# uzh-rpg/rpg_svo

Measured on AMD Instinct MI355X. Metric: frames/sec sparse-align+pose-refine (VGA, 4 pyr lvls); ATE vs CPU ref, higher is better.
Workload: dtype value = default build: K1 f32 pixels/residuals/chi2/per-pixel products, f64 Jacobian rows/partials/reductions/projection/solve/pose; K4 f64 (reference-width build: roofline_f64_build.value)

## Files before the change

rpg_svo_amd/csrc/pyr_addr.h:

```cpp
#pragma once
#include <stdint.h>

#ifndef SVO_HOST_MATH_TEST
#include <hip/hip_runtime.h>
#endif

namespace svo_pyr {

constexpr int TILE_W = 16, TILE_H = 8;

__host__ __device__ __forceinline__ uint32_t mul24(uint32_t a, uint32_t b) {
#ifdef __HIP_DEVICE_COMPILE__
  return __umul24(a, b);
#else
  return a * b;
#endif
}

__host__ __device__ __forceinline__ uint32_t row_off(int y, int pitch) {
  return mul24((uint32_t)(y >> 3), ((uint32_t)pitch << 3) - 128u) + ((uint32_t)y << 4);
}
__host__ __device__ __forceinline__ uint32_t col_off(int x) {
  return mul24((uint32_t)(x >> 4), 112u) + (uint32_t)x;
}
__host__ __device__ __forceinline__ uint32_t px_off(int x, int y, int pitch) { return row_off(y, pitch) + col_off(x); }

__host__ __device__ __forceinline__ int64_t level_bytes(int pitch, int h) {
  return (int64_t)pitch * ((h + 7) & ~7);
}


__device__ __forceinline__ int run_start(int c, int need) {
  int xa = c & ~3;
  if ((xa & 15) == 8 && (c & 15) + need <= 16) xa -= 4;
  return xa;
}

typedef uint32_t u32x2_t __attribute__((ext_vector_type(2)));
typedef uint32_t u32x3_t __attribute__((ext_vector_type(3)));
__device__ __forceinline__ uint32_t ld32(const uint8_t* __restrict__ lvl, uint32_t off) {
  return *reinterpret_cast<const uint32_t*>(lvl + off);
}
__device__ __forceinline__ u32x2_t ld64(const uint8_t* __restrict__ lvl, uint32_t off) {
  typedef u32x2_t __attribute__((aligned(4))) u32x2_a4;
  return *reinterpret_cast<const u32x2_a4*>(lvl + off);
}
__device__ __forceinline__ u32x3_t ld96(const uint8_t* __restrict__ lvl, uint32_t off) {
  typedef u32x3_t __attribute__((aligned(4))) u32x3_a4;
  return *reinterpret_cast<const u32x3_a4*>(lvl + off);
}

__device__ __forceinline__ void load_run12(const uint8_t* __restrict__ lvl, uint32_t ro, int xa, uint32_t d[3]) {
  const uint32_t a = ro + col_off(xa);
  const int o = xa & 15;
  if (o <= 4) {
    const u32x3_t v = ld96(lvl, a);
    d[0] = v.x; d[1] = v.y; d[2] = v.z;
  } else if (o == 8) {
    const u32x2_t v = ld64(lvl, a);
    d[0] = v.x; d[1] = v.y;
    d[2] = ld32(lvl, a + 120u);
  } else {
    d[0] = ld32(lvl, a);
    const u32x2_t v = ld64(lvl, a + 116u);
    d[1] = v.x; d[2] = v.y;
  }
}

template <int NR>
__device__ __forceinline__ void load_window12(const uint8_t* __restrict__ lvl, int pitch, int xa, int v0,
                                              uint32_t d[][3]) {
  uint32_t a[NR];
  const uint32_t c = col_off(xa);
#pragma unroll
  for (int r = 0; r < NR; ++r) a[r] = row_off(v0 + r, pitch) + c;
  const int o = xa & 15;
  if (o <= 4) {
#pragma unroll
    for (int r = 0; r < NR; ++r) {
      const u32x3_t v = ld96(lvl, a[r]);
      d[r][0] = v.x; d[r][1] = v.y; d[r][2] = v.z;
    }
  } else if (o == 8) {
#pragma unroll
    for (int r = 0; r < NR; ++r) {
      const u32x2_t v = ld64(lvl, a[r]);
      d[r][0] = v.x; d[r][1] = v.y;
      d[r][2] = ld32(lvl, a[r] + 120u);
    }
  } else {
#pragma unroll
    for (int r = 0; r < NR; ++r) {
      d[r][0] = ld32(lvl, a[r]);
      const u32x2_t v = ld64(lvl, a[r] + 116u);
      d[r][1] = v.x; d[r][2] = v.y;
    }
  }
}

}
```

rpg_svo_amd/csrc/sia_common.h:

```cpp
#pragma once
#include "capi_common.h"
#include "device_math.h"
#include "track_math.h"
#include "wave_reduce.h"

namespace svo_sia {

using namespace svo_capi;
using namespace svo_dev;

struct SiaArgs {
  svo_hip_pyr_layout L;
  const uint8_t* store;
  const int32_t* ref_slot;
  const int32_t* cur_slot;
  const int32_t* n;
  int n_stride;
  const double* px;
  const double* xyz;
  const uint8_t* valid;
  svo_hip_sia_params P;
  const double* T_in;
  double* T_out;
  double* H_out;
  int32_t* n_tracked;
  int32_t* iters;
  double* chi2;
  int32_t* status;
  int B = 0;
  void* xw = nullptr;
};

struct XChunk {
  unsigned lo, tag0, hi, tag1;
};
static_assert(sizeof(XChunk) == 16, "one 16-byte access");
constexpr int SIA_X_SLOTS = 16;
constexpr int SIA_XH_SLOTS = 24;
constexpr int SIA_X_MAX_PARTS = 4;
constexpr int SIA_X_CHUNKS = 2 * SIA_X_MAX_PARTS * (SIA_X_SLOTS + SIA_XH_SLOTS);
constexpr int SIA_X_BLOCK = SIA_X_CHUNKS + 1;

#ifndef SVO_HOST_MATH_TEST
__device__ __forceinline__ void sia_xstore(XChunk* p, double v, unsigned epoch) {
  typedef unsigned int u4 __attribute__((ext_vector_type(4)));
  const unsigned long long b = (unsigned long long)__double_as_longlong(v);
  u4 w;
  w.x = (unsigned)b; w.y = epoch; w.z = (unsigned)(b >> 32); w.w = epoch;
  asm volatile("global_store_dwordx4 %0, %1, off sc1\n\ts_nop 3" ::"v"(p), "v"(w) : "memory");
}
__device__ __forceinline__ XChunk sia_xload(const XChunk* p) {
  typedef unsigned int u4 __attribute__((ext_vector_type(4)));
  u4 w;
  asm volatile("global_load_dwordx4 %0, %1, off sc1\n\ts_waitcnt vmcnt(0)" : "=v"(w) : "v"(p) : "memory");
  XChunk c;
  c.lo = w.x; c.tag0 = w.y; c.hi = w.z; c.tag1 = w.w;
  return c;
}
__device__ __forceinline__ void sia_xstore_epoch(XChunk* p, unsigned epoch) {
  typedef unsigned int u4 __attribute__((ext_vector_type(4)));
  u4 w;
  w.x = epoch; w.y = 0u; w.z = 0u; w.w = 0u;
  asm volatile("global_store_dwordx4 %0, %1, off sc1\n\ts_nop 3" ::"v"(p), "v"(w) : "memory");
}
__device__ __forceinline__ double sia_xpoll(const XChunk* p, unsigned epoch, int& failed) {
  XChunk c = sia_xload(p);
  unsigned spins = 0;
  while (c.tag0 != epoch || c.tag1 != epoch) {
    if (++spins > (1u << 16)) {
      failed = 1;
      return __longlong_as_double(0x7ff8000000000000ll);
    }
    __builtin_amdgcn_s_sleep(1);
    c = sia_xload(p);
  }
  return __longlong_as_double((long long)(((unsigned long long)c.hi << 32) | c.lo));
}
#endif

using svo_pyr::load_window12;
using svo_pyr::run_start;


__device__ __forceinline__ void cut_row7(const uint32_t d[3], uint32_t bo, float out[7]) {
  const bool up = bo >= 4u;
  const uint32_t a = up ? d[1] : d[0], b = up ? d[2] : d[1], c = up ? 0u : d[2];
  const uint32_t sel = bo & 3u;
  const uint32_t lo = __builtin_amdgcn_alignbyte(b, a, sel);
  const uint32_t hi = __builtin_amdgcn_alignbyte(c, b, sel);
  out[0] = (float)(lo & 0xffu);
  out[1] = (float)((lo >> 8) & 0xffu);
  out[2] = (float)((lo >> 16) & 0xffu);
  out[3] = (float)(lo >> 24);
  out[4] = (float)(hi & 0xffu);
  out[5] = (float)((hi >> 8) & 0xffu);
  out[6] = (float)((hi >> 16) & 0xffu);
}

__device__ __forceinline__ void cut_row5_plain(const uint32_t d[3], uint32_t bo, float out[5]) {
  const bool up = bo >= 4u;
  const uint32_t a = up ? d[1] : d[0], b = up ? d[2] : d[1];
  const uint32_t sel = bo & 3u;
  const uint32_t lo = __builtin_amdgcn_alignbyte(b, a, sel);
  const uint32_t hi = b >> (8 * sel);
  out[0] = (float)(lo & 0xffu);
  out[1] = (float)((lo >> 8) & 0xffu);
  out[2] = (float)((lo >> 16) & 0xffu);
  out[3] = (float)(lo >> 24);
  out[4] = (float)(hi & 0xffu);
}

__device__ __forceinline__ double sia_rcp(double z) {
  double r = __builtin_amdgcn_rcp(z);
  r = fma(fma(-z, r, 1.0), r, r);
  r = fma(fma(-z, r, 1.0), r, r);
  return r;
}

__device__ __forceinline__ uint32_t sel_e64(uint64_t mask, uint32_t if_set, uint32_t if_clear) {
#ifdef SIA_VCC_SELECT
  return ((mask >> (threadIdx.x & 63)) & 1) ? if_set : if_clear;
#else
  uint32_t r;
  asm("v_cndmask_b32_e64 %0, %1, %2, %3" : "=v"(r) : "v"(if_clear), "v"(if_set), "s"(mask));
  return r;
#endif
}
__device__ __forceinline__ void cut_row5(uint32_t a, uint32_t b, uint32_t c, int bo, uint64_t up, float out[5]) {
  const uint32_t d0 = sel_e64(up, b, a), d1 = sel_e64(up, c, b);
  const uint32_t sel = (uint32_t)(bo & 3);
  const uint32_t lo = __builtin_amdgcn_alignbyte(d1, d0, sel);
  const uint32_t hi = d1 >> (8 * sel);
  out[0] = (float)(lo & 0xffu);
  out[1] = (float)((lo >> 8) & 0xffu);
  out[2] = (float)((lo >> 16) & 0xffu);
  out[3] = (float)(lo >> 24);
  out[4] = (float)(hi & 0xffu);
}

__device__ __forceinline__ double sia_uni(double v) {
  const unsigned long long u = (unsigned long long)__double_as_longlong(v);
  const unsigned lo = (unsigned)__builtin_amdgcn_readfirstlane((int)(unsigned)u);
  const unsigned hi = (unsigned)__builtin_amdgcn_readfirstlane((int)(unsigned)(u >> 32));
  return __longlong_as_double((long long)(((unsigned long long)hi << 32) | lo));
}


__device__ __forceinline__ int sym6_rt(int i, int j) {
  const int a = i < j ? i : j, b = i < j ? j : i;
  return a * 6 - (a * (a - 1)) / 2 + (b - a);
}

int launch_sia_wave(const SiaArgs& args, int B, hipStream_t s);
bool sia_wave_applies(const SiaArgs& args, int B);

}
```

rpg_svo_amd/csrc/sparse_align.hip:

```cpp
#include <cstdlib>
#include <map>
#include <mutex>
#include <utility>

#include "sia_common.h"

using namespace svo_capi;
using namespace svo_dev;
using namespace svo_sia;

namespace {

#define MINW(BLOCK) ((BLOCK) >= 256 ? 4 : 3)

#ifdef SIA_PROFILE
#define SIA_T() ((long long)__builtin_readcyclecounter())
#define SIA_ACC(k, t0, t1) prof[k] += (t1) - (t0)
#else
#define SIA_T() 0ll
#define SIA_ACC(k, t0, t1)
#endif

constexpr int MAX_WAVES = SVO_HIP_MAX_PATCHES / 64;

// ... 6 lines not shown
using sia_pix = float;
using sia_acc = double;
#endif

struct SplitModel {
  double q[2][4], t[2][3];
};

struct SiaLds {
  SplitModel sm;
  double Rt[12];
  int sw_done, sw_stop, sw_nmeas, sw_cur, sw_old;
  double sw_chi2;
  double H[21];
  double Hinv[36];
  double A[36];
  sia_acc part[2][MAX_WAVES][8];
  int chg[2][MAX_WAVES];
  int xfail;
  sia_acc Hpart[MAX_WAVES][24];
  long long lo[SVO_HIP_MAX_LEVELS];
  int lw[SVO_HIP_MAX_LEVELS];
  int lh[SVO_HIP_MAX_LEVELS];
  int lp[SVO_HIP_MAX_LEVELS];
};
__shared__ SiaLds g_s;


template <int PARTS>
__device__ __forceinline__ void sia_rebuild_hinv(int lane, int nw, [[maybe_unused]] XChunk* xh, [[maybe_unused]] int part,
                                                 [[maybe_unused]] unsigned gen, [[maybe_unused]] int& xfail) {
  asm volatile("" : "+v"(lane));
#ifndef SVO_HOST_MATH_TEST
  if constexpr (PARTS > 1) {
    static_assert((PARTS - 1) * 21 <= 64, "one lane per chunk of the other parts");
    const int j = lane / 21, k = lane - 21 * j;
    double v = 0.0;
    for (int w = 0; w < nw; ++w) v += (double)g_s.Hpart[w][k];
    if (j == 0) sia_xstore(xh + part * SIA_XH_SLOTS + k, v, gen);
    const int other = j < part ? j : j + 1;
    double got = 0.0;
    if (j < PARTS - 1) got = sia_xpoll(xh + other * SIA_XH_SLOTS + k, gen, xfail);
    if (xfail) g_s.xfail = 1;
    double tot = 0.0;
#pragma unroll
    for (int p = 0; p < PARTS; ++p) {
      const double theirs = __shfl(got, (p < part ? p : p - 1) * 21 + k, 64);
      const double term = p == part ? v : theirs;
      tot = p == 0 ? term : tot + term;
    }
    if (lane < 21) g_s.H[lane] = tot;
  } else
#endif
  if (lane < 21) {
    double v = 0.0;
    for (int w = 0; w < nw; ++w) v += (double)g_s.Hpart[w][lane];
    g_s.H[lane] = v;
  }
  SVO_WAVE_LDS_FENCE();
  const int gi = lane / 6, gj = lane - 6 * gi;
  if (lane < 36) {
    g_s.A[lane] = g_s.H[sym6_rt(gi, gj)];
    g_s.Hinv[lane] = (gi == gj) ? 1.0 : 0.0;
  }
  for (int k = 0; k < 6; ++k) {
    SVO_WAVE_LDS_FENCE();
    if (lane < 36) {
      const double p = g_s.A[k * 6 + k];
      const double aik = g_s.A[gi * 6 + k];
      const double akj = g_s.A[k * 6 + gj];
      const double bkj = g_s.Hinv[k * 6 + gj];
      const double aij = g_s.A[lane];
      const double bij = g_s.Hinv[lane];
      const double ip = (fabs(p) > 2.2250738585072014e-308) ? sia_rcp(p) : 0.0;
      const double na = (gi == k) ? akj * ip : aij - aik * (akj * ip);
      const double nb = (gi == k) ? bkj * ip : bij - aik * (bkj * ip);
      SVO_LANES_LDS_FENCE();
      g_s.A[lane] = na;
      g_s.Hinv[lane] = nb;
    }
  }
}


__device__ __forceinline__ float sia_bilerp(float wtl, float wtr, float wbl, float wbr, float tl, float tr, float bl, float br) {
  return __builtin_fmaf(wbr, br, __builtin_fmaf(wbl, bl, __builtin_fmaf(wtr, tr, wtl * tl)));
}
typedef float sia_f2 __attribute__((ext_vector_type(2)));
__device__ __forceinline__ sia_f2 sia_bilerp2(sia_f2 wtl, sia_f2 wtr, sia_f2 wbl, sia_f2 wbr, sia_f2 tl, sia_f2 tr, sia_f2 bl,
                                              sia_f2 br) {
  return __builtin_elementwise_fma(wbr, br, __builtin_elementwise_fma(wbl, bl, __builtin_elementwise_fma(wtr, tr, wtl * tl)));
}

#ifdef SIA_F64_PARTIALS
#define SIA_PACKED 0
#else
#define SIA_PACKED 1
#endif
template <int BLOCK, bool WC, bool DIST, int PARTS = 1>
__global__ void __launch_bounds__(BLOCK, PARTS > 1 ? 1 : ((DIST && BLOCK < 1024) ? 3 : MINW(BLOCK))) sia_kernel(const SiaArgs a) {
  constexpr int NW = BLOCK / 64;
  int b, part = 0;
  if constexpr (PARTS > 1) {
    b = (int)(blockIdx.x / (8 * PARTS)) * 8 + (int)(blockIdx.x % 8);
    part = (int)(blockIdx.x / 8) % PARTS;
    if (b >= a.B) return;
  } else {
    b = (int)xcd_contiguous_block();
  }
  [[maybe_unused]] XChunk* const xbase = PARTS > 1 ? static_cast<XChunk*>(a.xw) + (size_t)b * SIA_X_BLOCK : nullptr;
  [[maybe_unused]] unsigned xseq = 0;
#ifndef SVO_HOST_MATH_TEST
  if constexpr (PARTS > 1) xseq = (unsigned)__builtin_amdgcn_readfirstlane((int)sia_xload(xbase + SIA_X_CHUNKS).lo);
#endif
  [[maybe_unused]] int xfail = 0;
  const int tid = threadIdx.x;
  const int lane = tid & 63;
  const int wave = tid >> 6;

  __shared__ float4 s_bt[8][BLOCK];

  int n = a.n[b];
  n = n > a.n_stride ? a.n_stride : n;
  const svo_hip_sia_params P = a.P;

  if (n <= 0) {
    if (tid == 0 && part == 0) {
      for (int k = 0; k < 12; ++k) a.T_out[12 * b + k] = a.T_in[12 * b + k];
      if (a.H_out)
        for (int k = 0; k < 36; ++k) a.H_out[36 * b + k] = 0.0;
      a.n_tracked[b] = 0;
      if (a.iters)
        for (int k = 0; k < SVO_HIP_MAX_LEVELS; ++k) a.iters[SVO_HIP_MAX_LEVELS * b + k] = 0;
      if (a.chi2) a.chi2[b] = 1e10;
      if (a.status) a.status[b] = 0;
    }
    return;
  }

  const int pid = part * BLOCK + tid;
  const size_t fo = (size_t)b * a.n_stride + pid;
  const bool has = (pid < n) && (a.valid ? a.valid[fo] != 0 : true);
  double X = 0, Y = 0, Z = 1;
  if (has) {
    X = a.xyz[3 * fo];
    Y = a.xyz[3 * fo + 1];
    Z = a.xyz[3 * fo + 2];
  }
  double px_kept0 = 0, px_kept1 = 0;
  if (has) {
    px_kept0 = a.px[2 * fo];
    px_kept1 = a.px[2 * fo + 1];
  }
  const double rz = sia_rcp(Z);
  const sia_acc zi = (sia_acc)rz;
  const sia_acc xn = (sia_acc)(X * rz);
  const sia_acc yn = (sia_acc)(Y * rz);
  const uint8_t* ref_base = a.store + (int64_t)a.ref_slot[b] * a.L.slot_bytes;
  const uint8_t* cur_base = a.store + (int64_t)a.cur_slot[b] * a.L.slot_bytes;

  if (tid == 0) {
#pragma unroll
    for (int k = 0; k < SVO_HIP_MAX_LEVELS; ++k) {
      g_s.lw[k] = a.L.w[k];
      g_s.lh[k] = a.L.h[k];
      g_s.lp[k] = a.L.pitch[k];
      g_s.lo[k] = a.L.offset[k];
    }
    for (int k = 0; k < 21; ++k) g_s.H[k] = 0.0;
    g_s.xfail = 0;
    if (a.iters && part == 0)
      for (int k = 0; k < SVO_HIP_MAX_LEVELS; ++k) a.iters[SVO_HIP_MAX_LEVELS * b + k] = 0;
  }
  double R[9], tr[3];
  {
    double q[4];
    for (int k = 0; k < 9; ++k) R[k] = a.T_in[12 * b + k];
    for (int k = 0; k < 3; ++k) tr[k] = a.T_in[12 * b + 9 + k];
    quat_from_R(R, q);
    quat_to_R(q, R);
    if (tid == 0) {
      for (int k = 0; k < 4; ++k) g_s.sm.q[0][k] = q[k];
      for (int k = 0; k < 3; ++k) g_s.sm.t[0][k] = tr[k];
    }
  }
  int m_cur = 0, m_old = 0;
  double chi2_prev = 1e10;
  int stop = 0;
  int n_meas_last = 0;
  int buf = 0;

  const int sw = (NW > 1) ? (int)(blockIdx.x % NW) : 0;
  sia_pix Sxx = 0, Sxy = 0, Syy = 0;
  sia_acc gmask = 0;
  bool vis = false;

  __syncthreads();

#ifdef SIA_PROFILE
  long long prof[8] = {0, 0, 0, 0, 0, 0, 0, 0};
  const long long t_begin = SIA_T();
#endif
  for (int level = P.max_level; level >= P.min_level; --level) {
    [[maybe_unused]] const long long tl0 = SIA_T();
    const int cols = g_s.lw[level], rows = g_s.lh[level], pitch = g_s.lp[level];
    const uint8_t* ref_img = ref_base + g_s.lo[level];
    const uint8_t* cur_img = cur_base + g_s.lo[level];
    const float scale = pow2_inv_f32(level);
    const sia_acc fl = (sia_acc)(fabs(P.fx) * pow2_inv_f64(level));

    uint32_t wc[WC ? 7 : 1][3];
    int wc_u0 = 0, wc_v0 = -100000;
    if (WC) {
#pragma unroll
      for (int r = 0; r < (WC ? 7 : 1); ++r) wc[r][0] = wc[r][1] = wc[r][2] = 0u;
    }
    {
      const double pxx = px_kept0, pxy = px_kept1;
      const float u_ref = (float)(pxx * (double)scale);
      const float v_ref = (float)(pxy * (double)scale);
      const int u_i = (int)floorf(u_ref);
      const int v_i = (int)floorf(v_ref);
      const bool inb = has && !(u_i - 3 < 0 || v_i - 3 < 0 || u_i + 3 >= cols || v_i + 3 >= rows);
      Sxx = Sxy = Syy = 0;
      if (inb) {
        vis = true;
        gmask = 1;
        const float su = u_ref - (float)u_i, sv = v_ref - (float)v_i;
        const float wtl = (1.f - su) * (1.f - sv);
        const float wtr = su * (1.f - sv);
        const float wbl = (1.f - su) * sv;
        const float wbr = su * sv;
        float Bt[6][6];
        float Wp[7], Wc[7];
        uint32_t rw[7][3];
        const int rxa = run_start(u_i - 3, 7);
        const uint32_t rbo = (uint32_t)(u_i - 3 - rxa);
        load_window12<7>(ref_img, pitch, rxa, v_i - 3, rw);
        cut_row7(rw[0], rbo, Wp);
#pragma unroll
        for (int r = 0; r < 6; ++r) {
          cut_row7(rw[r + 1], rbo, Wc);
#pragma unroll
          for (int c = 0; c < 6; ++c) {
            const bool need = ((r >= 1 && r <= 4)) || ((c >= 1 && c <= 4));
            if (need) Bt[r][c] = sia_bilerp(wtl, wtr, wbl, wbr, Wp[c], Wp[c + 1], Wc[c], Wc[c + 1]);
          }
#pragma unroll
          for (int c = 0; c < 7; ++c) Wp[c] = Wc[c];
        }
#pragma unroll
        for (int y = 0; y < 4; ++y)
#pragma unroll
          for (int x = 0; x < 4; ++x) {
            const float dx = 0.5f * (Bt[y + 1][x + 2] - Bt[y + 1][x]);
            const float dy = 0.5f * (Bt[y + 2][x + 1] - Bt[y][x + 1]);
            Sxx += (sia_pix)dx * (sia_pix)dx;
            Sxy += (sia_pix)dx * (sia_pix)dy;
            Syy += (sia_pix)dy * (sia_pix)dy;
          }
#if SIA_PACKED
        s_bt[0][tid] = make_float4(Bt[0][1], Bt[0][3], Bt[0][2], Bt[0][4]);
        s_bt[1][tid] = make_float4(Bt[1][0], Bt[1][2], Bt[1][1], Bt[1][3]);
        s_bt[2][tid] = make_float4(Bt[1][4], Bt[1][5], Bt[2][0], Bt[2][2]);
        s_bt[3][tid] = make_float4(Bt[2][1], Bt[2][3], Bt[2][4], Bt[2][5]);
        s_bt[4][tid] = make_float4(Bt[3][0], Bt[3][2], Bt[3][1], Bt[3][3]);
        s_bt[5][tid] = make_float4(Bt[3][4], Bt[3][5], Bt[4][0], Bt[4][2]);
        s_bt[6][tid] = make_float4(Bt[4][1], Bt[4][3], Bt[4][4], Bt[4][5]);
        s_bt[7][tid] = make_float4(Bt[5][1], Bt[5][3], Bt[5][2], Bt[5][4]);
#else
        s_bt[0][tid] = make_float4(Bt[0][1], Bt[0][2], Bt[0][3], Bt[0][4]);
        s_bt[1][tid] = make_float4(Bt[1][0], Bt[1][1], Bt[1][2], Bt[1][3]);
        s_bt[2][tid] = make_float4(Bt[1][4], Bt[1][5], Bt[2][0], Bt[2][1]);
        s_bt[3][tid] = make_float4(Bt[2][2], Bt[2][3], Bt[2][4], Bt[2][5]);
        s_bt[4][tid] = make_float4(Bt[3][0], Bt[3][1], Bt[3][2], Bt[3][3]);
        s_bt[5][tid] = make_float4(Bt[3][4], Bt[3][5], Bt[4][0], Bt[4][1]);
        s_bt[6][tid] = make_float4(Bt[4][2], Bt[4][3], Bt[4][4], Bt[4][5]);
        s_bt[7][tid] = make_float4(Bt[5][1], Bt[5][2], Bt[5][3], Bt[5][4]);
#endif
      } else {
        gmask = 0;
      }
    }

    m_old = m_cur;
    int inH = -1;
    int evals = 0;
    SIA_ACC(5, tl0, SIA_T());
    for (int iter = 0; iter < P.n_iter; ++iter) {
      [[maybe_unused]] const long long tp0 = SIA_T();
      bool m = false;
      sia_pix gx = 0, gy = 0;
      float c2 = 0.f;
      if (vis) {
        const double xc = R[0] * X + R[1] * Y + R[2] * Z + tr[0];
        const double yc = R[3] * X + R[4] * Y + R[5] * Z + tr[1];
        const double zc = R[6] * X + R[7] * Y + R[8] * Z + tr[2];
        double izc = __builtin_amdgcn_rcp(zc);
        izc = fma(fma(-zc, izc, 1.0), izc, izc);
        izc = fma(fma(-zc, izc, 1.0), izc, izc);
        double pu, pv;
        if (DIST) {
          Cam cm;
          cm.fx = P.fx; cm.fy = P.fy; cm.cx = P.cx; cm.cy = P.cy;
          cm.width = 0; cm.height = 0;
          cm.model = P.cam_model;
#pragma unroll
          for (int k = 0; k < 5; ++k) cm.d[k] = P.d[k];
          const double uvn[2] = {xc * izc, yc * izc};
          double pxd[2];
          world2cam_uv(cm, uvn, pxd);
          pu = pxd[0];
          pv = pxd[1];
        } else {
          pu = P.fx * (xc * izc) + P.cx;
          pv = P.fy * (yc * izc) + P.cy;
        }
        const float u_cur = (float)pu * scale;
        const float v_cur = (float)pv * scale;
        const float fu = floorf(u_cur), fv = floorf(v_cur);
        if (fu - 3.f >= 0.f && fv - 3.f >= 0.f && fu + 3.f < (float)cols && fv + 3.f < (float)rows) {
          m = true;
          const int u_i = (int)fu, v_i = (int)fv;
          const float su = u_cur - fu, sv = v_cur - fv;
          const float wtl = (1.f - su) * (1.f - sv);
          const float wtr = su * (1.f - sv);
          const float wbl = (1.f - su) * sv;
          const float wbr = su * sv;
          {
#if SIA_PACKED
          typedef float f2 __attribute__((ext_vector_type(2)));
          uint32_t cw[5][3];
          uint32_t cbo = 0;
          uint64_t k0 = 0, k1 = 0, kup = 0;
          int bo = 0;
          if (WC) {
            int r0 = (v_i - 2) - wc_v0;
            bo = (u_i - 2) - wc_u0;
            if (!(r0 >= 0 && r0 <= 2 && bo >= 0 && bo <= 7)) {
              wc_v0 = v_i - 3;
              wc_u0 = run_start(u_i - 3, 7);
              load_window12<(WC ? 7 : 1)>(cur_img, pitch, wc_u0, wc_v0, wc);
              r0 = 1;
              bo = (u_i - 2) - wc_u0;
            }
            k0 = SVO_BALLOT_ACTIVE(r0 == 0);
            k1 = SVO_BALLOT_ACTIVE(r0 == 1);
            kup = SVO_BALLOT_ACTIVE(bo >= 4);
          } else {
            const int cxa = run_start(u_i - 2, 5);
            cbo = (uint32_t)(u_i - 2 - cxa);
            load_window12<5>(cur_img, pitch, cxa, v_i - 2, cw);
          }
#define SIA_WIN_ROW(r, p02, p13, p24)                                                                                   \
  do {                                                                                                                  \
    float o_[5];                                                                                                        \
    if (WC) {                                                                                                           \
      constexpr int S_ = WC ? 1 : 0;                                                                                    \
      const uint32_t d0_ = sel_e64(k0, wc[(r) * S_][0], sel_e64(k1, wc[((r) + 1) * S_][0], wc[((r) + 2) * S_][0]));     \
      const uint32_t d1_ = sel_e64(k0, wc[(r) * S_][1], sel_e64(k1, wc[((r) + 1) * S_][1], wc[((r) + 2) * S_][1]));     \
      const uint32_t d2_ = sel_e64(k0, wc[(r) * S_][2], sel_e64(k1, wc[((r) + 1) * S_][2], wc[((r) + 2) * S_][2]));     \
      cut_row5(d0_, d1_, d2_, bo, kup, o_);                                                                             \
    } else {                                                                                                            \
      cut_row5_plain(cw[WC ? 0 : (r)], cbo, o_);                                                                        \
    }                                                                                                                   \
    p02 = f2{o_[0], o_[2]};                                                                                             \
    p13 = f2{o_[1], o_[3]};                                                                                             \
    p24 = f2{o_[2], o_[4]};                                                                                             \
  } while (0)
          const float2* const bt2 = reinterpret_cast<const float2*>(&s_bt[0][0]);
#define SIA_BT2(q, h) bt2[((q) * BLOCK + tid) * 2 + (h)]
          const f2 vtl = f2{wtl, wtl}, vtr = f2{wtr, wtr}, vbl = f2{wbl, wbl}, vbr = f2{wbr, wbr};
          f2 c2v = f2{0.f, 0.f}, gxv = f2{0.f, 0.f}, gyv = f2{0.f, 0.f};
          f2 t02, t13, t24, b02, b13, b24;
          SIA_WIN_ROW(0, t02, t13, t24);
          SIA_WIN_ROW(1, b02, b13, b24);
          f2 a13, a24, b02t, b13t, b45t, c02, c13, c45;
          { const float2 v0 = SIA_BT2(0, 0), v1 = SIA_BT2(0, 1); a13 = f2{v0.x, v0.y}; a24 = f2{v1.x, v1.y}; }
          { const float2 v0 = SIA_BT2(1, 0), v1 = SIA_BT2(1, 1), v2 = SIA_BT2(2, 0);
            b02t = f2{v0.x, v0.y}; b13t = f2{v1.x, v1.y}; b45t = f2{v2.x, v2.y}; }
          { const float2 v0 = SIA_BT2(2, 1), v1 = SIA_BT2(3, 0), v2 = SIA_BT2(3, 1);
            c02 = f2{v0.x, v0.y}; c13 = f2{v1.x, v1.y}; c45 = f2{v2.x, v2.y}; }
#pragma unroll
          for (int y = 0; y < 4; ++y) {
            f2 n02 = f2{0.f, 0.f}, n13 = f2{0.f, 0.f}, n45 = f2{0.f, 0.f};
            if (y == 0) { const float2 v0 = SIA_BT2(4, 0), v1 = SIA_BT2(4, 1), v2 = SIA_BT2(5, 0);
                          n02 = f2{v0.x, v0.y}; n13 = f2{v1.x, v1.y}; n45 = f2{v2.x, v2.y}; }
            if (y == 1) { const float2 v0 = SIA_BT2(5, 1), v1 = SIA_BT2(6, 0), v2 = SIA_BT2(6, 1);
                          n02 = f2{v0.x, v0.y}; n13 = f2{v1.x, v1.y}; n45 = f2{v2.x, v2.y}; }
            if (y == 2) { const float2 v0 = SIA_BT2(7, 0), v1 = SIA_BT2(7, 1);
                          n13 = f2{v0.x, v0.y}; n45 = f2{v1.x, v1.y}; }
            const f2 b24t = f2{b02t.y, b45t.x}, b35t = f2{b13t.y, b45t.y};
            const f2 c24 = (y < 3) ? f2{c02.y, c45.x} : c45;
            const f2 Ia = sia_bilerp2(vtl, vtr, vbl, vbr, t02, t13, b02, b13);
            const f2 Ib = sia_bilerp2(vtl, vtr, vbl, vbr, t13, t24, b13, b24);
            const f2 ra = Ia - b13t, rb = Ib - b24t;
            c2v += ra * ra;
            c2v += rb * rb;
            gxv += ra * (b24t - b02t);
            gxv += rb * (b35t - b13t);
            gyv += ra * (c13 - a13);
            gyv += rb * (c24 - a24);
            if (y < 3) {
              f2 w02, w13, w24;
              SIA_WIN_ROW(y + 2, w02, w13, w24);
              t02 = b02; t13 = b13; t24 = b24;
              b02 = w02; b13 = w13; b24 = w24;
              a13 = b13t; a24 = b24t;
              b02t = c02; b13t = c13; b45t = c45;
              c02 = n02; c13 = n13; c45 = n45;
              asm volatile("" ::: "memory");
            }
          }
#undef SIA_WIN_ROW
#undef SIA_BT2
          c2 += c2v.x + c2v.y;
          gx += gxv.x + gxv.y;
          gy += gyv.x + gyv.y;
#else
          float W[5][5];
          if (WC) {
            int r0 = (v_i - 2) - wc_v0;
            int bo = (u_i - 2) - wc_u0;
            if (!(r0 >= 0 && r0 <= 2 && bo >= 0 && bo <= 7)) {
              wc_v0 = v_i - 3;
              wc_u0 = run_start(u_i - 3, 7);
              load_window12<(WC ? 7 : 1)>(cur_img, pitch, wc_u0, wc_v0, wc);
              r0 = 1;
              bo = (u_i - 2) - wc_u0;
            }
            const uint64_t k0 = SVO_BALLOT_ACTIVE(r0 == 0), k1 = SVO_BALLOT_ACTIVE(r0 == 1);
            const uint64_t kup = SVO_BALLOT_ACTIVE(bo >= 4);
#pragma unroll
            for (int r = 0; r < 5; ++r) {
              constexpr int S = WC ? 1 : 0;
              const uint32_t d0 = sel_e64(k0, wc[r * S][0], sel_e64(k1, wc[(r + 1) * S][0], wc[(r + 2) * S][0]));
              const uint32_t d1 = sel_e64(k0, wc[r * S][1], sel_e64(k1, wc[(r + 1) * S][1], wc[(r + 2) * S][1]));
              const uint32_t d2 = sel_e64(k0, wc[r * S][2], sel_e64(k1, wc[(r + 1) * S][2], wc[(r + 2) * S][2]));
              cut_row5(d0, d1, d2, bo, kup, W[r]);
            }
          } else {
            uint32_t cw[5][3];
            const int cxa = run_start(u_i - 2, 5);
            const uint32_t cbo = (uint32_t)(u_i - 2 - cxa);
            load_window12<5>(cur_img, pitch, cxa, v_i - 2, cw);
#pragma unroll
            for (int r = 0; r < 5; ++r) cut_row5_plain(cw[r], cbo, W[r]);
          }
          float Bt[6][6];
          {
            const float4 q0 = s_bt[0][tid], q1 = s_bt[1][tid], q2 = s_bt[2][tid], q3 = s_bt[3][tid];
            const float4 q4 = s_bt[4][tid], q5 = s_bt[5][tid], q6 = s_bt[6][tid], q7 = s_bt[7][tid];
            Bt[0][0] = Bt[0][5] = Bt[5][0] = Bt[5][5] = 0.f;
            Bt[0][1] = q0.x; Bt[0][2] = q0.y; Bt[0][3] = q0.z; Bt[0][4] = q0.w;
            Bt[1][0] = q1.x; Bt[1][1] = q1.y; Bt[1][2] = q1.z; Bt[1][3] = q1.w;
            Bt[1][4] = q2.x; Bt[1][5] = q2.y; Bt[2][0] = q2.z; Bt[2][1] = q2.w;
            Bt[2][2] = q3.x; Bt[2][3] = q3.y; Bt[2][4] = q3.z; Bt[2][5] = q3.w;
            Bt[3][0] = q4.x; Bt[3][1] = q4.y; Bt[3][2] = q4.z; Bt[3][3] = q4.w;
            Bt[3][4] = q5.x; Bt[3][5] = q5.y; Bt[4][0] = q5.z; Bt[4][1] = q5.w;
            Bt[4][2] = q6.x; Bt[4][3] = q6.y; Bt[4][4] = q6.z; Bt[4][5] = q6.w;
            Bt[5][1] = q7.x; Bt[5][2] = q7.y; Bt[5][3] = q7.z; Bt[5][4] = q7.w;
          }
#pragma unroll
          for (int y = 0; y < 4; ++y)
#pragma unroll
            for (int x = 0; x < 4; ++x) {
              const float I = sia_bilerp(wtl, wtr, wbl, wbr, W[y][x], W[y][x + 1], W[y + 1][x], W[y + 1][x + 1]);
              const float res = I - Bt[y + 1][x + 1];
              c2 += res * res;
              gx += (sia_pix)res * (sia_pix)(Bt[y + 1][x + 2] - Bt[y + 1][x]);
              gy += (sia_pix)res * (sia_pix)(Bt[y + 2][x + 1] - Bt[y][x + 1]);
            }
#endif
          }
        }
      }
      {
        const sia_acc gsc = (sia_acc)0.5 * fl * gmask;
        const sia_acc gxf = m ? (sia_acc)gx * gsc : (sia_acc)0, gyf = m ? (sia_acc)gy * gsc : (sia_acc)0;
        sia_acc part[8];
        sia_acc zi_ = zi, xn_ = xn, yn_ = yn;
        asm volatile("" : "+v"(zi_), "+v"(xn_), "+v"(yn_));
        part[0] = zi_ * gxf;
        part[1] = zi_ * gyf;
        part[2] = -zi_ * (xn_ * gxf + yn_ * gyf);
        part[3] = -(xn_ * yn_ * gxf + ((sia_acc)1 + yn_ * yn_) * gyf);
        part[4] = ((sia_acc)1 + xn_ * xn_) * gxf + xn_ * yn_ * gyf;
        part[5] = xn_ * gyf - yn_ * gxf;
        part[6] = (sia_acc)c2;
        part[7] = m ? (sia_acc)16 : (sia_acc)0;
        [[maybe_unused]] const long long tp1 = SIA_T();
        SIA_ACC(0, tp0, tp1);
        const sia_acc tot = wave_reduce8(part, lane);
        if ((lane & 7) == 0) g_s.part[buf][wave][lane >> 3] = tot;
        const int mine = __builtin_amdgcn_ballot_w64((int)m != inH) != 0ull;
        if (lane == 0) g_s.chg[buf][wave] = mine;
        SIA_ACC(1, tp1, SIA_T());
      }
      [[maybe_unused]] const long long tb0 = SIA_T();
      __syncthreads();
      int changed = 0;
#pragma unroll
      for (int w = 0; w < NW; ++w) changed |= g_s.chg[buf][w];
      [[maybe_unused]] double xtot = 0.0;
#ifndef SVO_HOST_MATH_TEST
      if constexpr (PARTS > 1) {
        ++xseq;
        const int xp = lane >> 4, xk = lane & 15;
        double own = 0.0;
        if (xk < 8) {
#pragma unroll
          for (int w = 0; w < NW; ++w) own += (double)g_s.part[buf][w][xk];
        } else if (xk == 8) {
          own = (double)changed;
        }
        XChunk* const slot = xbase + (size_t)(xseq & 1) * (SIA_X_MAX_PARTS * SIA_X_SLOTS);
        if (wave == sw && xp == part && xk < 9) sia_xstore(slot + part * SIA_X_SLOTS + xk, own, xseq);
        double val = own;
        if (xp != part && xp < PARTS && xk < 9) val = sia_xpoll(slot + xp * SIA_X_SLOTS + xk, xseq, xfail);
        if (xfail) g_s.xfail = 1;
        xtot = __shfl(val, xk, 64);
#pragma unroll
        for (int p = 1; p < PARTS; ++p) xtot += __shfl(val, 16 * p + xk, 64);
        changed = readlane_f64<8>(xtot) != 0.0;
      }
#endif
      [[maybe_unused]] const long long tb1 = SIA_T();
      SIA_ACC(2, tb0, tb1);
      if (changed) {
        sia_acc zi_ = zi, xn_ = xn, yn_ = yn;
        asm volatile("" : "+v"(zi_), "+v"(xn_), "+v"(yn_));
        const sia_acc one = 1, zero = 0;
        const sia_acc ja[6] = {-zi_ * fl, zero, xn_ * zi_ * fl, xn_ * yn_ * fl, -(one + xn_ * xn_) * fl, yn_ * fl};
        const sia_acc jb[6] = {zero, -zi_ * fl, yn_ * zi_ * fl, (one + yn_ * yn_) * fl, -xn_ * yn_ * fl, -xn_ * fl};
        sia_acc hp[24];
#pragma unroll
        for (int i = 0; i < 6; ++i)
#pragma unroll
          for (int j = i; j < 6; ++j) {
            const sia_acc v = (sia_acc)Sxx * (ja[i] * ja[j]) + (sia_acc)Sxy * (ja[i] * jb[j] + jb[i] * ja[j]) + (sia_acc)Syy * (jb[i] * jb[j]);
            hp[sym6(i, j)] = m ? v : zero;
          }
        hp[21] = hp[22] = hp[23] = zero;
#pragma unroll
        for (int g = 0; g < 3; ++g) {
          const sia_acc tot = wave_reduce8(hp + 8 * g, lane);
          if ((lane & 7) == 0) g_s.Hpart[wave][8 * g + (lane >> 3)] = tot;
        }
        inH = (int)m;
        __syncthreads();
        if constexpr (PARTS > 1) {
          ++xseq;
          XChunk* const xh = xbase + 2 * SIA_X_MAX_PARTS * SIA_X_SLOTS + (size_t)(xseq & 1) * (SIA_X_MAX_PARTS * SIA_XH_SLOTS);
          if (wave == 0) sia_rebuild_hinv<PARTS>(lane, NW, xh, part, xseq, xfail);
        } else {
          if (wave == 0) sia_rebuild_hinv<1>(lane, NW, nullptr, 0, 0u, xfail);
        }
        __syncthreads();
      }
      ++evals;
      [[maybe_unused]] const long long ts0 = SIA_T();
      SIA_ACC(3, tb1, ts0);
#ifdef SIA_PROFILE
      prof[7] += 1;
#endif

      int done = 0;
      const int swb = (NW > 1) ? (sw + 1) % NW : sw;
      const bool rot_wave = wave == sw, trans_wave = wave == swb;
      int m_next = m_cur;
      if (rot_wave || trans_wave) {
        __builtin_amdgcn_s_setprio(3);
        double colsum = 0.0;
        if constexpr (PARTS > 1) {
          colsum = xtot;
        } else {
          const int k = lane & 7;
#pragma unroll
          for (int w = 0; w < NW; ++w) colsum += (double)g_s.part[buf][w][k];
        }
        const double b0 = readlane_f64<0>(colsum), b1 = readlane_f64<1>(colsum), b2 = readlane_f64<2>(colsum);
        const double b3 = readlane_f64<3>(colsum), b4 = readlane_f64<4>(colsum), b5 = readlane_f64<5>(colsum);
        const float chi2_sum = (float)readlane_f64<6>(colsum);
        const int n_meas = (int)readlane_f64<7>(colsum);
        double xi;
        {
          const double* row = &g_s.Hinv[6 * (lane < 6 ? lane : 0)];
          xi = row[0] * b0 + row[1] * b1 + row[2] * b2 + row[3] * b3 + row[4] * b4 + row[5] * b5;
        }
        const double x0 = readlane_f64<0>(xi), x1 = readlane_f64<1>(xi), x2 = readlane_f64<2>(xi);
        const double x3 = readlane_f64<3>(xi), x4 = readlane_f64<4>(xi), x5 = readlane_f64<5>(xi);
        n_meas_last = n_meas;
        const double new_chi2 = (double)(chi2_sum / (float)n_meas);
        if (isnan(x0)) stop = 1;
        const SplitModel& sm = g_s.sm;
        const bool rollback = (iter > 0 && new_chi2 > chi2_prev) || stop;
        if (rollback) {
          m_next = m_old;
          done = 1;
        } else {
          m_next = m_cur ^ 1;
          m_old = m_cur;
          chi2_prev = new_chi2;
          const double nm = fmax(fmax(fmax(fabs(x0), fabs(x1)), fmax(fabs(x2), fabs(x3))), fmax(fabs(x4), fabs(x5)));
          if (nm <= P.eps) done = 1;
        }
        const float mx[6] = {-(float)x0, -(float)x1, -(float)x2, -(float)x3, -(float)x4, -(float)x5};
        if (rot_wave) {
          double q[4];
          if (rollback) {
#pragma unroll
            for (int k = 0; k < 4; ++k) q[k] = sm.q[m_next][k];
          } else {
#ifdef SIA_F64_PARTIALS
            const double mxd[6] = {-x0, -x1, -x2, -x3, -x4, -x5};
            double eq[4], et_unused[3];
            se3_exp(mxd, eq, et_unused);
#else
            float eqf[4];
            se3_exp_rot_f32(mx, eqf);
            const double eq[4] = {eqf[0], eqf[1], eqf[2], eqf[3]};
#endif
            double oq[4];
#pragma unroll
            for (int k = 0; k < 4; ++k) oq[k] = sm.q[m_cur][k];
            quat_mul(oq, eq, q);
            quat_normalize_fast(q);
            if (lane == 0) {
#pragma unroll
              for (int k = 0; k < 4; ++k) g_s.sm.q[m_next][k] = q[k];
            }
          }
          quat_to_R(q, R);
          if (lane == 0) {
#pragma unroll
            for (int k = 0; k < 9; ++k) g_s.Rt[k] = R[k];
            g_s.sw_done = done;
            g_s.sw_stop = stop;
            g_s.sw_nmeas = n_meas_last;
            g_s.sw_chi2 = chi2_prev;
            g_s.sw_cur = m_next;
            g_s.sw_old = m_old;
          }
        }
        if (trans_wave) {
          if (rollback) {
#pragma unroll
            for (int k = 0; k < 3; ++k) tr[k] = sm.t[m_next][k];
          } else {
#ifdef SIA_F64_PARTIALS
            const double mxd[6] = {-x0, -x1, -x2, -x3, -x4, -x5};
            double eq_unused[4], et[3];
            se3_exp(mxd, eq_unused, et);
#else
            float etf[3];
            se3_exp_trans_f32(mx, etf);
            const double et[3] = {etf[0], etf[1], etf[2]};
#endif
            double oq[4], rt[3];
#pragma unroll
            for (int k = 0; k < 4; ++k) oq[k] = sm.q[m_cur][k];
            quat_rot(oq, et, rt);
#pragma unroll
            for (int k = 0; k < 3; ++k) tr[k] = sm.t[m_cur][k] + rt[k];
            if (lane == 0) {
#pragma unroll
              for (int k = 0; k < 3; ++k) g_s.sm.t[m_next][k] = tr[k];
            }
          }
          if (lane == 0) {
#pragma unroll
            for (int k = 0; k < 3; ++k) g_s.Rt[9 + k] = tr[k];
          }
        }
        __builtin_amdgcn_s_setprio(0);
      }
      m_cur = m_next;
      if (NW > 1) {
        __syncthreads();
#pragma unroll
        for (int k = 0; k < 9; ++k) R[k] = g_s.Rt[k];
#pragma unroll
        for (int k = 0; k < 3; ++k) tr[k] = g_s.Rt[9 + k];
        done = g_s.sw_done;
        stop = g_s.sw_stop;
        n_meas_last = g_s.sw_nmeas;
        chi2_prev = g_s.sw_chi2;
        m_cur = g_s.sw_cur;
        m_old = g_s.sw_old;
      }
      buf ^= 1;
      SIA_ACC(4, ts0, SIA_T());
      if (done) break;
    }
    if (tid == 0 && part == 0 && a.iters) a.iters[SVO_HIP_MAX_LEVELS * b + level] = evals;
  }

  if (tid == 0 && part == 0) {
    for (int k = 0; k < 9; ++k) a.T_out[12 * b + k] = R[k];
    for (int k = 0; k < 3; ++k) a.T_out[12 * b + 9 + k] = tr[k];
    if (a.H_out)
      for (int i = 0; i < 6; ++i)
        for (int j = 0; j < 6; ++j) a.H_out[36 * b + i * 6 + j] = g_s.H[sym6_rt(i, j)];
#ifdef SIA_PROFILE
    prof[6] = SIA_T() - t_begin;
    if (a.H_out)
      for (int k = 0; k < 8; ++k) a.H_out[36 * b + k] = (double)prof[k];
#endif
    a.n_tracked[b] = n_meas_last / 16;
    if (a.chi2) a.chi2[b] = chi2_prev;
    if constexpr (PARTS > 1) {
#ifndef SVO_HOST_MATH_TEST
      sia_xstore_epoch(xbase + SIA_X_CHUNKS, xseq + (g_s.xfail ? (1u << 16) : 0u));
#endif
    }
    if (a.status) a.status[b] = (stop ? SVO_HIP_SIA_STOP : 0) | ((PARTS > 1 && g_s.xfail) ? SVO_HIP_SIA_EXCHANGE_TIMEOUT : 0);
  }
}


template <int BLOCK>
int launch(const SiaArgs& args, int B, hipStream_t s) {
  constexpr bool WC = BLOCK == 256;
  if (args.P.cam_model == SVO_HIP_CAM_PINHOLE)
    hipLaunchKernelGGL((sia_kernel<BLOCK, WC, false>), dim3(B), dim3(BLOCK), 0, s, args);
  else
    hipLaunchKernelGGL((sia_kernel<BLOCK, false, true>), dim3(B), dim3(BLOCK), 0, s, args);
  return check_launch();
}

}

namespace {

int sia_prepare(const svo_hip_pyr_layout* layout, const uint8_t* d_store, int B, const int32_t* d_ref_slot,
                const int32_t* d_cur_slot, const int32_t* d_n, int n_stride, const double* d_px, const double* d_xyz_ref,
                const uint8_t* d_valid, const svo_hip_sia_params* params, const double* d_T_in, double* d_T_out,
                double* d_H_out, int32_t* d_n_tracked, int32_t* d_iters, double* d_chi2, int32_t* d_status, SiaArgs* out) {
  if (!layout_ok(layout) || !d_store || !params || B < 0) return SVO_HIP_EINVAL;
  if (B == 0) return SVO_HIP_OK;
  if (!d_ref_slot || !d_cur_slot || !d_n || !d_px || !d_xyz_ref || !d_T_in || !d_T_out || !d_n_tracked)
    return SVO_HIP_EINVAL;
  if (n_stride < 1) return SVO_HIP_EINVAL;
  if (n_stride > SVO_HIP_MAX_PATCHES) return SVO_HIP_ERANGE;
  if (params->min_level < 0 || params->max_level < params->min_level || params->max_level >= layout->n_levels ||
      params->n_iter < 0)
    return SVO_HIP_EINVAL;
  if (params->cam_model != SVO_HIP_CAM_PINHOLE && params->cam_model != SVO_HIP_CAM_PINHOLE_RADTAN &&
      params->cam_model != SVO_HIP_CAM_ATAN)
    return SVO_HIP_EINVAL;
  SiaArgs& args = *out;
  args.L = *layout;
  args.store = d_store;
  args.ref_slot = d_ref_slot;
  args.cur_slot = d_cur_slot;
  args.n = d_n;
  args.n_stride = n_stride;
  args.px = d_px;
  args.xyz = d_xyz_ref;
  args.valid = d_valid;
  args.P = *params;
  args.T_in = d_T_in;
  args.T_out = d_T_out;
  args.H_out = d_H_out;
  args.n_tracked = d_n_tracked;
  args.iters = d_iters;
  args.chi2 = d_chi2;
  args.status = d_status;
  return 1;
}

constexpr int SIA_SPLIT_PARTS = 4;
constexpr int SIA_SPLIT_MAX_B = 128;
#ifndef SVO_HOST_MATH_TEST
bool sia_split_applies(const SiaArgs& args, int B) {
  static const bool on = [] { const char* v = std::getenv("SVO_HIP_K1_SPLIT"); return !(v && v[0] == '0'); }();
  return on && args.n_stride > 512 && B <= SIA_SPLIT_MAX_B;
}
void* sia_split_blocks(hipStream_t s) {
  static std::mutex mut;
  static std::map<std::pair<int, hipStream_t>, void*> blocks;
  int dev = 0;
  if (hipGetDevice(&dev) != hipSuccess) return nullptr;
// ... 71 lines not shown
```

Before: 11.54 million.

## Hoist level-start projection, window fetch and Hessian build ahead of the iteration loop

At each pyramid level start, the kernel now projects the point, fetches both the reference and current 7-row windows with a branch-free flat loader, and builds and reduces the per-wave Hessian partials before the first iteration. Iteration 0 reuses that projection and skips its own Hessian rebuild. Several LDS-loaded scalars are forced uniform with readfirstlane, kept pixel coordinates move to f32, and gmask becomes a bool. The goal is to overlap memory latency with setup work and remove redundant first-iteration work, at the cost of extra register pressure and unconditional loads for invisible points.

```diff
diff --git a/rpg_svo_amd/csrc/pyr_addr.h b/rpg_svo_amd/csrc/pyr_addr.h
--- a/rpg_svo_amd/csrc/pyr_addr.h
+++ b/rpg_svo_amd/csrc/pyr_addr.h
@@ -98,4 +98,27 @@
   }
 }
 
+template <int NR>
+__device__ __forceinline__ void load_window12_flat(const uint8_t* __restrict__ lvl, int pitch, int xa, int v0,
+                                                   uint32_t d[][3]) {
+  const int o = xa & 15;
+  const uint32_t c = col_off(xa);
+  const uint32_t ca = o == 12 ? c + 116u : c;
+  const uint32_t cb = o <= 4 ? c + 8u : (o == 8 ? c + 120u : c);
+  u32x2_t A[NR];
+  uint32_t B[NR];
+#pragma unroll
+  for (int r = 0; r < NR; ++r) {
+    const uint32_t ro = row_off(v0 + r, pitch);
+    A[r] = ld64(lvl, ro + ca);
+    B[r] = ld32(lvl, ro + cb);
+  }
+#pragma unroll
+  for (int r = 0; r < NR; ++r) {
+    d[r][0] = o == 12 ? B[r] : A[r].x;
+    d[r][1] = o == 12 ? A[r].x : A[r].y;
+    d[r][2] = o == 12 ? A[r].y : B[r];
+  }
 }
+
+}
diff --git a/rpg_svo_amd/csrc/sia_common.h b/rpg_svo_amd/csrc/sia_common.h
--- a/rpg_svo_amd/csrc/sia_common.h
+++ b/rpg_svo_amd/csrc/sia_common.h
@@ -79,6 +79,7 @@
 #endif
 
 using svo_pyr::load_window12;
+using svo_pyr::load_window12_flat;
 using svo_pyr::run_start;
 
 
@@ -144,7 +145,7 @@
   const unsigned hi = (unsigned)__builtin_amdgcn_readfirstlane((int)(unsigned)(u >> 32));
   return __longlong_as_double((long long)(((unsigned long long)hi << 32) | lo));
 }
-
+__device__ __forceinline__ int sia_uni_i32(int v) { return __builtin_amdgcn_readfirstlane(v); }
 
 __device__ __forceinline__ int sym6_rt(int i, int j) {
   const int a = i < j ? i : j, b = i < j ? j : i;
diff --git a/rpg_svo_amd/csrc/sparse_align.hip b/rpg_svo_amd/csrc/sparse_align.hip
--- a/rpg_svo_amd/csrc/sparse_align.hip
+++ b/rpg_svo_amd/csrc/sparse_align.hip
@@ -112,6 +112,56 @@
   }
 }
 
+#define SIA_STRINGIFY_(x) #x
+#define SIA_STRINGIFY(x) SIA_STRINGIFY_(x)
+constexpr bool SIA_LEVEL_START_JOINT = sizeof(SIA_STRINGIFY(SIA_LEVEL_START_SPLIT)) == sizeof("SIA_LEVEL_START_SPLIT");
+
+__device__ __forceinline__ void sia_project_pinhole(const double R[9], const double tr[3], double X, double Y, double Z,
+                                                    const svo_hip_sia_params& P, double& pu, double& pv) {
+  const double xc = R[0] * X + R[1] * Y + R[2] * Z + tr[0];
+  const double yc = R[3] * X + R[4] * Y + R[5] * Z + tr[1];
+  const double zc = R[6] * X + R[7] * Y + R[8] * Z + tr[2];
+  double izc = __builtin_amdgcn_rcp(zc);
+  izc = fma(fma(-zc, izc, 1.0), izc, izc);
+  izc = fma(fma(-zc, izc, 1.0), izc, izc);
+  pu = P.fx * (xc * izc) + P.cx;
+  pv = P.fy * (yc * izc) + P.cy;
+}
+
+template <bool APART>
+__device__ __forceinline__ void sia_store_hpart(sia_acc zi_, sia_acc xn_, sia_acc yn_, sia_acc fl, sia_pix Sxx, sia_pix Sxy,
+                                                sia_pix Syy, bool m, int lane, int wave) {
+  const sia_acc one = 1, zero = 0;
+  sia_acc hp[24];
+  sia_acc tie = zero;
+#pragma unroll
+  for (int g = 0; g < 3; ++g) {
+    if (APART) asm volatile("" : "+v"(zi_), "+v"(xn_), "+v"(yn_), "+v"(tie));
+    const sia_acc ja[6] = {-zi_ * fl, zero, xn_ * zi_ * fl, xn_ * yn_ * fl, -(one + xn_ * xn_) * fl, yn_ * fl};
+    const sia_acc jb[6] = {zero, -zi_ * fl, yn_ * zi_ * fl, (one + yn_ * yn_) * fl, -xn_ * yn_ * fl, -xn_ * fl};
+#pragma unroll
+    for (int i = 0; i < 6; ++i)
+#pragma unroll
+      for (int j = i; j < 6; ++j) {
+        if (sym6(i, j) / 8 != g) continue;
+        const sia_acc v = (sia_acc)Sxx * (ja[i] * ja[j]) + (sia_acc)Sxy * (ja[i] * jb[j] + jb[i] * ja[j]) + (sia_acc)Syy * (jb[i] * jb[j]);
+        hp[sym6(i, j)] = m ? v : zero;
+      }
+    if (g == 2) hp[21] = hp[22] = hp[23] = zero;
+    if (APART) {
+      tie = wave_reduce8(hp + 8 * g, lane);
+      if ((lane & 7) == 0) g_s.Hpart[wave][8 * g + (lane >> 3)] = tie;
+    }
+  }
+  if (!APART) {
+#pragma unroll
+    for (int g = 0; g < 3; ++g) {
+      const sia_acc tot = wave_reduce8(hp + 8 * g, lane);
+      if ((lane & 7) == 0) g_s.Hpart[wave][8 * g + (lane >> 3)] = tot;
+    }
+  }
+}
+
 
 __device__ __forceinline__ float sia_bilerp(float wtl, float wtr, float wbl, float wbr, float tl, float tr, float bl, float br) {
   return __builtin_fmaf(wbr, br, __builtin_fmaf(wbl, bl, __builtin_fmaf(wtr, tr, wtl * tl)));
@@ -130,6 +180,8 @@
 template <int BLOCK, bool WC, bool DIST, int PARTS = 1>
 __global__ void __launch_bounds__(BLOCK, PARTS > 1 ? 1 : ((DIST && BLOCK < 1024) ? 3 : MINW(BLOCK))) sia_kernel(const SiaArgs a) {
   constexpr int NW = BLOCK / 64;
+  constexpr bool LS_FETCH = WC && !DIST && SIA_LEVEL_START_JOINT;
+  constexpr bool LS_PROJ = LS_FETCH, LS_HPART = LS_FETCH;
   int b, part = 0;
   if constexpr (PARTS > 1) {
     b = (int)(blockIdx.x / (8 * PARTS)) * 8 + (int)(blockIdx.x % 8);
@@ -177,10 +229,10 @@
     Y = a.xyz[3 * fo + 1];
     Z = a.xyz[3 * fo + 2];
   }
-  double px_kept0 = 0, px_kept1 = 0;
+  float px_kept0 = 0.f, px_kept1 = 0.f;
   if (has) {
-    px_kept0 = a.px[2 * fo];
-    px_kept1 = a.px[2 * fo + 1];
+    px_kept0 = (float)a.px[2 * fo];
+    px_kept1 = (float)a.px[2 * fo + 1];
   }
   const double rz = sia_rcp(Z);
   const sia_acc zi = (sia_acc)rz;
@@ -212,6 +264,8 @@
     if (tid == 0) {
       for (int k = 0; k < 4; ++k) g_s.sm.q[0][k] = q[k];
       for (int k = 0; k < 3; ++k) g_s.sm.t[0][k] = tr[k];
+      for (int k = 0; k < 9; ++k) g_s.Rt[k] = R[k];
+      for (int k = 0; k < 3; ++k) g_s.Rt[9 + k] = tr[k];
     }
   }
   int m_cur = 0, m_old = 0;
@@ -222,7 +276,7 @@
 
   const int sw = (NW > 1) ? (int)(blockIdx.x % NW) : 0;
   sia_pix Sxx = 0, Sxy = 0, Syy = 0;
-  sia_acc gmask = 0;
+  bool gmask = false;
   bool vis = false;
 
   __syncthreads();
@@ -233,29 +287,49 @@
 #endif
   for (int level = P.max_level; level >= P.min_level; --level) {
     [[maybe_unused]] const long long tl0 = SIA_T();
-    const int cols = g_s.lw[level], rows = g_s.lh[level], pitch = g_s.lp[level];
-    const uint8_t* ref_img = ref_base + g_s.lo[level];
-    const uint8_t* cur_img = cur_base + g_s.lo[level];
+    const int cols = sia_uni_i32(g_s.lw[level]), rows = sia_uni_i32(g_s.lh[level]), pitch = sia_uni_i32(g_s.lp[level]);
+    const long long lvl_off = __double_as_longlong(sia_uni(__longlong_as_double(g_s.lo[level])));
+    const uint8_t* ref_img = ref_base + lvl_off;
+    const uint8_t* cur_img = cur_base + lvl_off;
     const float scale = pow2_inv_f32(level);
     const sia_acc fl = (sia_acc)(fabs(P.fx) * pow2_inv_f64(level));
 
     uint32_t wc[WC ? 7 : 1][3];
     int wc_u0 = 0, wc_v0 = -100000;
-    if (WC) {
+    if (WC && !LS_FETCH) {
 #pragma unroll
       for (int r = 0; r < (WC ? 7 : 1); ++r) wc[r][0] = wc[r][1] = wc[r][2] = 0u;
     }
+    [[maybe_unused]] float ls_u = 0.f, ls_v = 0.f;
+    [[maybe_unused]] bool ls_m = false;
     {
-      const double pxx = px_kept0, pxy = px_kept1;
-      const float u_ref = (float)(pxx * (double)scale);
-      const float v_ref = (float)(pxy * (double)scale);
+      const float u_ref = px_kept0 * scale;
+      const float v_ref = px_kept1 * scale;
       const int u_i = (int)floorf(u_ref);
       const int v_i = (int)floorf(v_ref);
       const bool inb = has && !(u_i - 3 < 0 || v_i - 3 < 0 || u_i + 3 >= cols || v_i + 3 >= rows);
       Sxx = Sxy = Syy = 0;
+      uint32_t rw[7][3];
+      uint32_t rbo = 0;
+      if constexpr (LS_FETCH) {
+        const int ru = inb ? u_i : 3, rv = inb ? v_i : 3;
+        const int rxa = run_start(ru - 3, 7);
+        rbo = (uint32_t)(ru - 3 - rxa);
+        double pu, pv;
+        sia_project_pinhole(R, tr, X, Y, Z, P, pu, pv);
+        ls_u = (float)pu * scale;
+        ls_v = (float)pv * scale;
+        const float fu = floorf(ls_u), fv = floorf(ls_v);
+        ls_m = (vis || inb) && fu - 3.f >= 0.f && fv - 3.f >= 0.f && fu + 3.f < (float)cols && fv + 3.f < (float)rows;
+        const int cu = ls_m ? (int)fu : 3, cv = ls_m ? (int)fv : 3;
+        wc_u0 = run_start(cu - 3, 7);
+        load_window12_flat<7>(ref_img, pitch, rxa, rv - 3, rw);
+        load_window12_flat<(WC ? 7 : 1)>(cur_img, pitch, wc_u0, cv - 3, wc);
+        wc_v0 = ls_m ? cv - 3 : -100000;
+      }
       if (inb) {
         vis = true;
-        gmask = 1;
+        gmask = true;
         const float su = u_ref - (float)u_i, sv = v_ref - (float)v_i;
         const float wtl = (1.f - su) * (1.f - sv);
         const float wtr = su * (1.f - sv);
@@ -263,10 +337,11 @@
         const float wbr = su * sv;
         float Bt[6][6];
         float Wp[7], Wc[7];
-        uint32_t rw[7][3];
-        const int rxa = run_start(u_i - 3, 7);
-        const uint32_t rbo = (uint32_t)(u_i - 3 - rxa);
-        load_window12<7>(ref_img, pitch, rxa, v_i - 3, rw);
+        if constexpr (!LS_FETCH) {
+          const int rxa = run_start(u_i - 3, 7);
+          rbo = (uint32_t)(u_i - 3 - rxa);
+          load_window12<7>(ref_img, pitch, rxa, v_i - 3, rw);
+        }
         cut_row7(rw[0], rbo, Wp);
 #pragma unroll
         for (int r = 0; r < 6; ++r) {
@@ -309,12 +384,18 @@
         s_bt[7][tid] = make_float4(Bt[5][1], Bt[5][2], Bt[5][3], Bt[5][4]);
 #endif
       } else {
-        gmask = 0;
+        gmask = false;
       }
     }
 
     m_old = m_cur;
     int inH = -1;
+    if constexpr (LS_HPART) {
+      sia_acc zi_ = zi, xn_ = xn, yn_ = yn;
+      asm volatile("" : "+v"(zi_), "+v"(xn_), "+v"(yn_), "+v"(Sxx));
+      sia_store_hpart<true>(zi_, xn_, yn_, fl, Sxx, Sxy, Syy, ls_m, lane, wave);
+      inH = (int)ls_m;
+    }
     int evals = 0;
     SIA_ACC(5, tl0, SIA_T());
     for (int iter = 0; iter < P.n_iter; ++iter) {
@@ -323,31 +404,37 @@
       sia_pix gx = 0, gy = 0;
       float c2 = 0.f;
       if (vis) {
-        const double xc = R[0] * X + R[1] * Y + R[2] * Z + tr[0];
-        const double yc = R[3] * X + R[4] * Y + R[5] * Z + tr[1];
-        const double zc = R[6] * X + R[7] * Y + R[8] * Z + tr[2];
-        double izc = __builtin_amdgcn_rcp(zc);
-        izc = fma(fma(-zc, izc, 1.0), izc, izc);
-        izc = fma(fma(-zc, izc, 1.0), izc, izc);
-        double pu, pv;
-        if (DIST) {
-          Cam cm;
-          cm.fx = P.fx; cm.fy = P.fy; cm.cx = P.cx; cm.cy = P.cy;
-          cm.width = 0; cm.height = 0;
-          cm.model = P.cam_model;
-#pragma unroll
-          for (int k = 0; k < 5; ++k) cm.d[k] = P.d[k];
-          const double uvn[2] = {xc * izc, yc * izc};
-          double pxd[2];
-          world2cam_uv(cm, uvn, pxd);
-          pu = pxd[0];
-          pv = pxd[1];
+        float u_cur, v_cur;
+        if (LS_PROJ && iter == 0) {
+          u_cur = ls_u;
+          v_cur = ls_v;
+          asm volatile("" : "+v"(u_cur), "+v"(v_cur));
         } else {
-          pu = P.fx * (xc * izc) + P.cx;
-          pv = P.fy * (yc * izc) + P.cy;
-        }
-        const float u_cur = (float)pu * scale;
-        const float v_cur = (float)pv * scale;
+          double pu, pv;
+          if (DIST) {
+            const double xc = R[0] * X + R[1] * Y + R[2] * Z + tr[0];
+            const double yc = R[3] * X + R[4] * Y + R[5] * Z + tr[1];
+            const double zc = R[6] * X + R[7] * Y + R[8] * Z + tr[2];
+            double izc = __builtin_amdgcn_rcp(zc);
+            izc = fma(fma(-zc, izc, 1.0), izc, izc);
+            izc = fma(fma(-zc, izc, 1.0), izc, izc);
+            Cam cm;
+            cm.fx = P.fx; cm.fy = P.fy; cm.cx = P.cx; cm.cy = P.cy;
+            cm.width = 0; cm.height = 0;
+            cm.model = P.cam_model;
+#pragma unroll
+            for (int k = 0; k < 5; ++k) cm.d[k] = P.d[k];
+            const double uvn[2] = {xc * izc, yc * izc};
+            double pxd[2];
+            world2cam_uv(cm, uvn, pxd);
+            pu = pxd[0];
+            pv = pxd[1];
+          } else {
+            sia_project_pinhole(R, tr, X, Y, Z, P, pu, pv);
+          }
+          u_cur = (float)pu * scale;
+          v_cur = (float)pv * scale;
+        }
         const float fu = floorf(u_cur), fv = floorf(v_cur);
         if (fu - 3.f >= 0.f && fv - 3.f >= 0.f && fu + 3.f < (float)cols && fv + 3.f < (float)rows) {
           m = true;
@@ -506,7 +593,7 @@
         }
       }
       {
-        const sia_acc gsc = (sia_acc)0.5 * fl * gmask;
+        const sia_acc gsc = gmask ? (sia_acc)0.5 * fl : (sia_acc)0;
         const sia_acc gxf = m ? (sia_acc)gx * gsc : (sia_acc)0, gyf = m ? (sia_acc)gy * gsc : (sia_acc)0;
         sia_acc part[8];
         sia_acc zi_ = zi, xn_ = xn, yn_ = yn;
@@ -522,9 +609,11 @@
         [[maybe_unused]] const long long tp1 = SIA_T();
         SIA_ACC(0, tp0, tp1);
         const sia_acc tot = wave_reduce8(part, lane);
-        if ((lane & 7) == 0) g_s.part[buf][wave][lane >> 3] = tot;
+        int lane_ = lane, wave_ = wave;
+        asm volatile("" : "+v"(lane_), "+v"(wave_));
+        if ((lane_ & 7) == 0) g_s.part[buf][wave_][lane_ >> 3] = tot;
         const int mine = __builtin_amdgcn_ballot_w64((int)m != inH) != 0ull;
-        if (lane == 0) g_s.chg[buf][wave] = mine;
+        if (lane_ == 0) g_s.chg[buf][wave_] = mine;
         SIA_ACC(1, tp1, SIA_T());
       }
       [[maybe_unused]] const long long tb0 = SIA_T();
@@ -557,28 +646,15 @@
 #endif
       [[maybe_unused]] const long long tb1 = SIA_T();
       SIA_ACC(2, tb0, tb1);
-      if (changed) {
-        sia_acc zi_ = zi, xn_ = xn, yn_ = yn;
-        asm volatile("" : "+v"(zi_), "+v"(xn_), "+v"(yn_));
-        const sia_acc one = 1, zero = 0;
-        const sia_acc ja[6] = {-zi_ * fl, zero, xn_ * zi_ * fl, xn_ * yn_ * fl, -(one + xn_ * xn_) * fl, yn_ * fl};
-        const sia_acc jb[6] = {zero, -zi_ * fl, yn_ * zi_ * fl, (one + yn_ * yn_) * fl, -xn_ * yn_ * fl, -xn_ * fl};
-        sia_acc hp[24];
-#pragma unroll
-        for (int i = 0; i < 6; ++i)
-#pragma unroll
-          for (int j = i; j < 6; ++j) {
-            const sia_acc v = (sia_acc)Sxx * (ja[i] * ja[j]) + (sia_acc)Sxy * (ja[i] * jb[j] + jb[i] * ja[j]) + (sia_acc)Syy * (jb[i] * jb[j]);
-            hp[sym6(i, j)] = m ? v : zero;
-          }
-        hp[21] = hp[22] = hp[23] = zero;
-#pragma unroll
-        for (int g = 0; g < 3; ++g) {
-          const sia_acc tot = wave_reduce8(hp + 8 * g, lane);
-          if ((lane & 7) == 0) g_s.Hpart[wave][8 * g + (lane >> 3)] = tot;
-        }
-        inH = (int)m;
-        __syncthreads();
+      const bool first_h = LS_HPART && iter == 0 && !changed;
+      if (changed || first_h) {
+        if (!first_h) {
+          sia_acc zi_ = zi, xn_ = xn, yn_ = yn;
+          asm volatile("" : "+v"(zi_), "+v"(xn_), "+v"(yn_));
+          sia_store_hpart<false>(zi_, xn_, yn_, fl, Sxx, Sxy, Syy, m, lane, wave);
+          inH = (int)m;
+          __syncthreads();
+        }
         if constexpr (PARTS > 1) {
           ++xseq;
           XChunk* const xh = xbase + 2 * SIA_X_MAX_PARTS * SIA_X_SLOTS + (size_t)(xseq & 1) * (SIA_X_MAX_PARTS * SIA_XH_SLOTS);
@@ -712,12 +788,12 @@
         for (int k = 0; k < 9; ++k) R[k] = g_s.Rt[k];
 #pragma unroll
         for (int k = 0; k < 3; ++k) tr[k] = g_s.Rt[9 + k];
-        done = g_s.sw_done;
-        stop = g_s.sw_stop;
-        n_meas_last = g_s.sw_nmeas;
-        chi2_prev = g_s.sw_chi2;
-        m_cur = g_s.sw_cur;
-        m_old = g_s.sw_old;
+        done = sia_uni_i32(g_s.sw_done);
+        stop = sia_uni_i32(g_s.sw_stop);
+        n_meas_last = sia_uni_i32(g_s.sw_nmeas);
+        chi2_prev = sia_uni(g_s.sw_chi2);
+        m_cur = sia_uni_i32(g_s.sw_cur);
+        m_old = sia_uni_i32(g_s.sw_old);
       }
       buf ^= 1;
       SIA_ACC(4, ts0, SIA_T());
@@ -727,8 +803,7 @@
   }
 
   if (tid == 0 && part == 0) {
-    for (int k = 0; k < 9; ++k) a.T_out[12 * b + k] = R[k];
-    for (int k = 0; k < 3; ++k) a.T_out[12 * b + 9 + k] = tr[k];
+    for (int k = 0; k < 12; ++k) a.T_out[12 * b + k] = g_s.Rt[k];
     if (a.H_out)
       for (int i = 0; i < 6; ++i)
         for (int j = 0; j < 6; ++j) a.H_out[36 * b + i * 6 + j] = g_s.H[sym6_rt(i, j)];
```

Result: slower. 10.45 million (-9.5%).
